# pierluigiferrari/fcn8s_tensorflow

Hardware: AMD Instinct MI355X
Metric: training images/sec at 1024x512 bs16 (higher is better)
Workload: dtype f32; 1 GPU; FCN-8s (VGG-16, fc6 7x7, 20 classes) train step, 1024x512, 16 images/GPU, SGD+momentum, keep_prob 0.5; global_batch=16, parallelism=dp1

## Files before the change

fcn8s_tensorflow_amd/csrc/conv_route.h:

```cpp
#pragma once
#include <algorithm>

namespace fcn8s {

struct RouteOpts {
    int wino_min_cin = 64;
    int wino_tile = 6;
    int wino_tile_hires = 0, wino_hires_pixels = 0;
    int wino_force_tile = 0;
    int wino_fc6 = 1;
    int plan_N = 0;
    bool scratch = false;
};
struct ConvShape { int N, H, W, Cin, Cout, K; };
inline ConvShape transposed(ConvShape s) { std::swap(s.Cin, s.Cout); return s; }

inline int wino_tile_for(const RouteOpts& o, int H, int W, int K = 3)
{
    if (H % 2 || W % 2) return 0;
    if (o.wino_force_tile && K == 3) return (o.wino_force_tile == 6 || (H % o.wino_force_tile == 0 && W % o.wino_force_tile == 0)) ? o.wino_force_tile : 0;
    int tmax = o.wino_tile;
    if (K == 3 && o.wino_tile_hires && o.wino_hires_pixels > 0 && (long long)H * W >= o.wino_hires_pixels && o.wino_tile_hires < tmax) tmax = o.wino_tile_hires;
    const bool t4 = tmax >= 4 && H % 4 == 0 && W % 4 == 0;
    if (K == 7) return (o.wino_tile >= 4 && H % 4 == 0 && W % 4 == 0) ? 4 : 0;
// ... 29 lines not shown
inline RbWriter relu_record_writer(const RouteOpts& o, const ConvShape& l, const ConvShape& next, bool l_is_conv1_1)
{
    if (l_is_conv1_1 && l.Cout % 64 == 0 && keeps_v(o, next)) return RbWriter::consumer;
    return keeps_v(o, l) ? RbWriter::self : RbWriter::none;
}
inline bool out_in_fused(const RouteOpts& o, const ConvShape& l, const ConvShape& next) { return l.K == 3 && next.K == 3 && fwd_tile(o, l) == 6 && fwd_tile(o, next) == 6; }
inline bool conv1_in_next_transform(const RouteOpts& o, const ConvShape& conv1_1, const ConvShape& next) { return conv1_1.Cout == 64 && fwd_tile(o, next) == 6; }
inline bool dm_from_next(const RouteOpts& o, const ConvShape& l)
{
    return o.scratch && keeps_v(o, l) && wino_tile_for(o, l.H, l.W, 3) == 6 && l.Cin % 64 == 0 && l.Cout % 64 == 0;
}
inline bool pool_in_transform(const RouteOpts& o, const ConvShape& last, bool has_prev)
{
    return o.wino_min_cin > 0 && last.Cout >= o.wino_min_cin && o.scratch && wino_tile_for(o, last.H, last.W, 3) >= 4 && last.Cout % 64 == 0 && has_prev && keeps_v(o, last);
}

struct Bf16Opts {
    bool acts = true;
    bool fuse_pool = true;
    bool conv1_tiled = true;
    bool copies = true;
};
inline bool bf16_kernels_take(const ConvShape& s) { return s.Cin % 64 == 0 && s.Cout % 64 == 0 && s.K % 2 == 1; }
inline bool pool_feeds_skip(int block) { return block == 3 || block == 4; }
inline bool bf16_plane_fits(long long plane_elems) { return (double)plane_elems * 2.0 + 65536.0 < 4294967296.0; }

inline bool conv1_writes_bf16_only(const Bf16Opts& o, const ConvShape& conv1_1, const ConvShape& next)
{
    return o.copies && o.acts && o.conv1_tiled && conv1_1.H % 8 == 0 && conv1_1.W % 16 == 0 && conv1_1.Cout % 64 == 0 && bf16_kernels_take(next);
}
// ... 26 lines not shown
```

fcn8s_tensorflow_amd/csrc/fcn8s_internal.h:

```cpp
#pragma once
#include <hip/hip_runtime.h>
#include <stdint.h>
#include <cmath>
#include "../../include/fcn8s_hip.h"

#if defined(__HIP_DEVICE_COMPILE__) && !defined(__gfx950__)
#error "libfcn8s_hip is written for gfx950 (MI355X) only: build with --offload-arch=gfx950"
#endif
#define FCN8S_LDS_BYTES_NEEDED (160u * 1024u)

#include <string>
namespace fcn8s {

extern thread_local const char* g_last_kernel;
void defer_error(int code, const char* fmt, ...) __attribute__((format(printf, 2, 3)));
int take_deferred_error(std::string* text);

struct IgemmArgs {
    const float* x; const float* w; const float* bias; const float* addend; const float* mask;
    float* y;
    int N, Ma, Mb; long long M;
    int Hi, Wi, Cin, ldx;
    int KW, in_scale, tap_step, tap_off, Ktot;
    int Ho, Wo, Cout, ldy;
// ... 187 lines not shown
inline float tf_adam_lr_t(float lr, float b1, float b2, long long t)
{
    return lr * (float)std::sqrt(1.0 - std::pow((double)b2, (double)t)) / (float)(1.0 - std::pow((double)b1, (double)t));
}
void launch_ema_update(float* sh, const float* theta, long long n, float w, const int* ok_dev, hipStream_t s);
void launch_swap(float* a, float* b, long long n, hipStream_t s);
void launch_flip_transpose(const float* w, float* wt, int taps, int Cin, int Cout, hipStream_t s);
void launch_pad_cin(const float* w, float* w4, int taps, int Cin, int Cinp, int Cout, hipStream_t s);
void launch_tconv_phase_pack(const float* w, float* wp, int K, int S, int C, hipStream_t s);
void launch_dropout_mask(float* mask, long long n, float keep_prob, unsigned long long seed,
                         unsigned int stream_id, hipStream_t s);
int wino_r(int KS);
int wino_nsub(int KS);
int wino_alpha(int tile, int KS);
long long wino_slab(long long T, int C);
void launch_wino_filter(int tile, const float* w, float* u, int Cin, int Cout, int KS, hipStream_t s, int transpose_out = 0);
void launch_wino_input(int tile, const float* x, float* v, int N, int H, int W, int C, int KS, hipStream_t s, unsigned* rbits_out = nullptr);
void launch_wino_input_conv1(const float* x0, const float* w4, const float* bias, float* v, int N, int H, int W, hipStream_t s, unsigned* rbits_out = nullptr);
void launch_wino_input_xb(const float* x, float* v, unsigned short* xb, int N, int H, int W, int C, hipStream_t s, unsigned* rbits_out = nullptr);
bool launch_wino_input_dout(int tile, const float* dy, float* v, float* dm, int N, int H, int W, int C, hipStream_t s, const unsigned char* pidx = nullptr);
void launch_wino_output(int tile, const float* m, const float* bias, const float* addend, const float* mask, float mask_scale,
                        int relu, float* y, int N, int H, int W, int C, int dropout, float keep, unsigned long long seed,
                        unsigned int stream_id, hipStream_t s, float* pool = nullptr, unsigned char* pidx = nullptr, int KS = 3,
                        unsigned* rbits_out = nullptr, const unsigned* rbits_in = nullptr);
size_t wino_rbits_words(int tile, int N, int H, int W, int C);
void launch_wino_dout(int tile, const float* dy, float* dm, int N, int H, int W, int C, hipStream_t s, int KS = 3, const unsigned char* pidx = nullptr);
void launch_wino_dgrad_output_dout(const float* dv, const unsigned* rbits_in, float* dm, int N, int H, int W, int C, hipStream_t s);
void launch_wino_dgrad_output_sub44(const float* dv, float* dx, int N, int H, int W, int C, hipStream_t s);
void launch_wino_dgrad_output(const float* dv, const float* addend, const float* mask, float mask_scale, const unsigned* rbits_in, float* y,
                              int N, int H, int W, int C, hipStream_t s);
bool launch_wino_out_in(const float* m, const float* bias, float* v, unsigned* rbits_out, int N, int H, int W, int C, hipStream_t s, bool always = false);
// ... 81 lines not shown
```

fcn8s_tensorflow_amd/csrc/model.hip:

```cpp
#include "../../include/fcn8s_hip.h"
#include "fcn8s_internal.h"
#include "device_buffer.h"
#include "pass_state.h"
#include "conv_route.h"
#include <cstdarg>
#include <functional>

#include <dlfcn.h>
#include <atomic>
#include <chrono>
#include <thread>
#include <cmath>
#include <cstdio>
#include <cstring>
#include <cstdlib>
#include <algorithm>
#include <mutex>
#include <map>
#include <set>
#include <string>
#include <vector>

using namespace fcn8s;

// ... 31 lines not shown
struct Act { float* p = nullptr; size_t n = 0; int H = 0, W = 0, C = 0; };

const int kConvsPerBlock[5] = {2, 2, 3, 3, 3};

struct Layer {
    char name[8], pool_name[8], pool_in[12];
    int block, pos, nconv;
    int h, w, cin, cout, K, real_cin;
    int prev, next;
    size_t w_off, b_off;
    int i_y, i_rb, i_wv, i_pool, i_pidx;
    float *y, *wv, *pool; unsigned* rb; unsigned char* pidx;
    int tile;
    RbWriter rb_writer;
    bool out_in_next, conv1_in_next;
    bool dm_from_next, pool_in_transform;
    ConvShape shape(int N) const { return ConvShape{N, h, w, cin, cout, K}; }
    bool first() const { return real_cin != 0; }
    bool last_of_block() const { return pos == nconv; }
};

}

namespace fcn8s {
void defer_error(int code, const char* fmt, ...)
{
    if (t_deferred_code) return;
    char buf[1024];
    va_list ap; va_start(ap, fmt); vsnprintf(buf, sizeof buf, fmt, ap); va_end(ap);
    t_deferred_code = code; t_deferred_text = buf;
}
// ... 40 lines not shown
    int wino_tile_hires = 0, wino_hires_pixels = 0;
    int wino_force_tile = 0;
    int precision = FCN8S_PREC_F32;
    bool frozen = false;
    unsigned long long frozen_fp = 0; DeviceBuf<unsigned long long> d_fp;
    PinnedBuf<unsigned long long> h_fp; hipEvent_t fp_event = nullptr;
    std::map<std::string, DeviceBuf<float>> u_cache;
    std::map<std::string, DeviceBuf<float>> u_train;
    bool fwd_train = false;
    PassState pass;
    int deterministic = 0;
    int fuse_dgrad_dout = 1;
    int fuse_out_in = 1;
    int conv1_tiled = 1, conv1_wgrad_mfma = 1;
    int conv1_in_transform = 1;
    DeviceBuf<unsigned short> d_wbf16;
    std::map<std::string, DeviceBuf<unsigned short>> wbf16_cache;
    std::set<std::string> bank_stale; bool banks_stale = false;
    int bf16_gemm256 = 1;
    DeviceBuf<unsigned short> d_abf16;
    std::map<std::string, DeviceBuf<unsigned short>> xbf16;
    using G16Map = std::map<std::string, DeviceBuf<unsigned short>>;
    G16Map xg16, dyg16;
    std::set<std::string> g16_stale;
    int bf16_fuse_pool = 1;
    int bf16_infer_copies = 1;
    int bf16_rows_bn = 0;
    int bf16_acts = 1;
    bool fp8_calibrated = false; float fp8_amax[FCN8S_FP8_LAYERS] = {}; DeviceBuf<unsigned> d_fp8_amax;
    std::map<std::string, Q8Buf> q8;
// ... 182 lines not shown

static void prof_derived(fcn8s_model* m, const char* what)
{
    if (m && m->profile && m->profile_detail) m->groups[group_id(m, (std::string("derived:") + what).c_str())].launches += 1;
}

struct ConvEpi { float alpha = 1.f; };
struct FwdEpi : ConvEpi {
    const float* bias = nullptr; int relu = 0;
    int dropout = 0; float keep = 1.f; uint32_t stream_id = 0;
    float* pool_out = nullptr; unsigned char* pool_idx = nullptr;
    int skip_y = 0;
    unsigned* relu_bits_out = nullptr;
    unsigned* in_relu_bits_out = nullptr; const char* in_layer = nullptr;
    float* next_v = nullptr; const char* next_layer = nullptr;
};
struct DgradEpi : ConvEpi {
    const float* addend = nullptr;
    const float* mask = nullptr; float mask_scale = 1.f;
    const unsigned* relu_bits_in = nullptr;
    const float* w_fwd = nullptr;
    int lazy_wt = 0;
    float* dm_out = nullptr; const char* dm_out_layer = nullptr;
    const char* yb_layer = nullptr; int yb_K = 3;
    bool yb_only = false;
};

thread_local int t_op_split = 0;
thread_local int t_op_rows_bn = 0;
thread_local int t_op_planes = 1;
// ... 22 lines not shown
    o.wino_min_cin = m->wino_min_cin; o.wino_tile = m->wino_tile; o.wino_tile_hires = m->wino_tile_hires; o.wino_hires_pixels = m->wino_hires_pixels;
    o.wino_force_tile = m->wino_force_tile; o.wino_fc6 = m->wino_fc6; o.plan_N = m->plan_N; o.scratch = m->d_wino_v != nullptr;
    return o;
}
int wino_tile_for(const fcn8s_model* m, int H, int W, int K = 3) { return m ? wino_tile_for(route_opts(m), H, W, K) : 0; }
Bf16Opts bf16_opts(const fcn8s_model* m, bool train)
{
    Bf16Opts o; o.acts = m->bf16_acts != 0; o.fuse_pool = m->bf16_fuse_pool != 0; o.conv1_tiled = m->conv1_tiled != 0; o.copies = train || m->bf16_infer_copies != 0;
    return o;
}
long long wino_tiles(int tile, int N, int H, int W) { return (long long)N * ((H + tile - 1) / tile) * ((W + tile - 1) / tile); }
struct WinoEpi { const float* bias = nullptr; const float* addend = nullptr; const float* mask = nullptr; float mask_scale = 1.f;
                 int relu = 0; int dropout = 0; float keep = 1.f; unsigned long long seed = 0; unsigned int stream_id = 0; float* pool = nullptr; unsigned char* pidx = nullptr;
                 unsigned* rbits_out = nullptr; const unsigned* rbits_in = nullptr; int skip_y = 0;
                 unsigned* in_rbits_out = nullptr;
                 float* next_v = nullptr; bool* fused_out = nullptr; };
static bool fft6_cheaper(const fcn8s_model* m, int H, int W)
{
    const long long fft = 292LL * ((H + 7) / 8) * ((W + 7) / 8);
    const long long other = wino_tile_for(m, H, W, 7) == 4 ? 196LL * (H / 4) * (W / 4) : 49LL * H * W;
    return fft < other;
}
static bool fft6_shape_ok(const fcn8s_model* m, int ci, int co) { return m->wino_fc6 && m->fc6_fft && m->fc6k == 7 && ci % 16 == 0 && co % 128 == 0; }
static bool fft6_on(const fcn8s_model* m, int N, int H, int W, int ci, int co)
{
    if (!m || !fft6_shape_ok(m, ci, co) || !fft6_cheaper(m, H, W) || m->precision != FCN8S_PREC_F32 || m->frozen || !m->d_wino_v || !m->d_wino_m) return false;
    const long long T = fft_fc6_tiles(N, H, W);
    auto v = m->acts.find("wino_v"), mm = m->acts.find("wino_m");
    return v != m->acts.end() && mm != m->acts.end() && v->second.n >= (size_t)fft_fc6_planes() * (size_t)wino_slab(T, ci) &&
           mm->second.n >= std::max((size_t)fft_fc6_planes() * (size_t)wino_slab(T, co), (size_t)T * 196 * ci);
}
// ... 96 lines not shown
    a.fixed_tile = 1; a.bt = 1; a.ldw = Cdy;
    { ProfScope ps(m, "fc6_fft_gemm_dgrad", 2.0 * P * T * Cdy * Cdx, 4.0 * P * (T * (double)(Cdy + Cdx) + (double)Cdy * Cdx), layer); launch_igemm(a, P, s); }
    { ProfScope ps(m, "fc6_fft_transform", 0, 4.0 * ((double)P * T * Cdx + 2.0 * 196.0 * T * Cdx + (double)N * H * W * Cdx));
      launch_fft_fc6_din(m->d_wino_v, m->d_wino_m, dx, N, H, W, Cdx, s); }
}

void conv_winograd(fcn8s_model* m, int tile, int KS, bool fwd, const float* x, const float* wk, float* y, float* u, float* v, float* mm,
                   int N, int H, int W, int Cin, int Cout, const WinoEpi& e, hipStream_t s, const char* layer, bool v_ready = false)
{
    const int P = wino_alpha(tile, KS) * wino_alpha(tile, KS), nsub2 = wino_nsub(KS) * wino_nsub(KS);
    const long long T = wino_tiles(tile, N, H, W);
    const int Kg = nsub2 * Cin;
    IgemmArgs a = position_gemm(v, u, mm, T, Kg, Cout); a.split = split_of(m);
    const double tb = 4.0 * ((double)N * H * W * Cin * nsub2 + (double)P * T * Kg), ob = 4.0 * ((double)N * H * W * Cout * ((e.pool ? (e.skip_y ? 0.25 : 1.25) : 1.0) + (e.rbits_in ? 1.0 / 32 : (e.mask ? 1.0 : 0.0)) + (e.addend ? 1.0 : 0.0) + (e.rbits_out ? 1.0 / 32 : 0.0)) + (double)P * T * Cout);
    bool u_cached = false;
    const char* tag = KS == 7 ? (fwd ? "wino_gemm_fc6_fwd" : "wino_gemm_fc6_dgrad") : (fwd ? "wino_gemm_fwd" : "wino_gemm_dgrad");
    if (m && m->frozen && layer && fwd) {
        DeviceBuf<float>& cu = m->u_cache[std::string(layer) + "#" + std::to_string(tile)];
        const std::string key = "u:" + std::string(layer) + "#" + std::to_string(tile);
        if (cu && !m->bank_stale.count(key)) { u = cu; u_cached = true; }
        else if (cu) { u = cu; m->bank_stale.erase(key); }
        else if (cu.grow((size_t)P * Kg * Cout * sizeof(float), s, &m->ws_allocs)) u = cu;
        a.w = u;
    }
    if (m && !u_cached && m->fwd_train && layer && fwd && ((KS == 3 && tile == 6) || (KS == 7 && tile == 4))) {
        DeviceBuf<float>& tu = m->u_train[std::string(layer) + "#" + std::to_string(tile)];
        if (tu.grow((size_t)P * Kg * Cout * sizeof(float), s)) { u = tu; a.w = u; }
    }
    auto pre = [&]() { if (!u_cached) { prof_derived(m, "wino_filter_kernel"); launch_wino_filter(tile, wk, u, Cin, Cout, KS, s); } if (!v_ready) launch_wino_input(tile, x, v, N, H, W, Cin, KS, s, e.in_rbits_out); };
    auto post = [&]() {
        if (e.next_v && tile == 6 && KS == 3 && e.relu && e.bias && !e.addend && !e.mask && !e.dropout && !e.pool && !e.rbits_in &&
            launch_wino_out_in(mm, e.bias, e.next_v, e.rbits_out, N, H, W, Cout, s, m && m->fuse_out_in >= 2)) { if (e.fused_out) *e.fused_out = true; return; }
        launch_wino_output(tile, mm, e.bias, e.addend, e.mask, e.mask_scale, e.relu, (e.skip_y && e.pool) ? nullptr : y, N, H, W, Cout, e.dropout, e.keep, e.seed, e.stream_id, s, e.pool, e.pidx, KS, e.rbits_out, e.rbits_in); };
    const double ob_fused = 4.0 * (2.0 * P * T * Cout + (e.rbits_out ? (double)N * H * W * Cout / 32 : 0.0));
    { ProfScope ps(m, "wino_transform", 0, (v_ready ? 0.0 : tb) + (u_cached ? 0.0 : (double)(KS * KS + P * nsub2) * 4 * Cin * Cout)); pre(); }
    { ProfScope ps(m, tag, 2.0 * P * T * Kg * Cout, 4.0 * P * (T * (double)(Kg + Cout) + (double)Kg * Cout), layer); launch_igemm(a, P, s); }
    { ProfScope ps(m, "wino_transform", 0, ob); post(); if (e.fused_out && *e.fused_out && m && m->profile && !m->groups.empty()) { const int g = group_id(m, "wino_transform"); m->groups[g].bytes += ob_fused - ob; } }
}

static void conv_direct(fcn8s_model* m, const char* group, IgemmArgs a, const float* x, const float* w, float* y,
                        int N, int H, int W, int Cin, int Cout, int K, hipStream_t s, int real_cin, const char* layer)
{
    a.split = split_of(m);
    a.x = x; a.w = w; a.y = y;
    a.N = N; a.Ma = H; a.Mb = W; a.M = (long long)N * H * W;
    a.Hi = H; a.Wi = W; a.Cin = Cin; a.ldx = Cin;
    a.KW = K; a.in_scale = 1; a.tap_step = 1; a.tap_off = -(K - 1) / 2; a.Ktot = K * K * Cin;
    a.Ho = H; a.Wo = W; a.Cout = Cout; a.ldy = Cout;
    a.out_scale = 1; a.out_offy = 0; a.out_offx = 0; a.phases_x = 1; a.w_phase_stride = 0;
    a.seed = m ? m->seed : 0;
// ... 18 lines not shown
        conv_fft6_fwd(m, layer, x, w, y, N, H, W, Cin, Cout, e.bias, e.relu, e.dropout, e.keep, e.stream_id, s)) return false;
    if (m) m->pass.drop_backward_handoffs();
    const int tile = fwd_tile(route_opts(m), ConvShape{N, H, W, Cin, Cout, K});
    if (tile && !(K == 3 && e.dropout) && e.alpha == 1.f && !real_cin) {
        const bool v_ready = m->pass.fwd_v.take(layer);
        m->pass.fwd_v.drop();
        float* vbuf = m->d_wino_v;
        if (layer) { auto it = m->acts.find(std::string("wv:") + layer); if (it != m->acts.end()) vbuf = it->second.p; }
        WinoEpi we; we.bias = e.bias; we.relu = e.relu;
        we.dropout = e.dropout; we.keep = e.keep; we.seed = m->seed; we.stream_id = e.stream_id; we.pool = e.pool_out; we.pidx = e.pool_idx;
        we.rbits_out = e.relu_bits_out; we.skip_y = e.skip_y && e.pool_out;
        if (e.relu_bits_out && layer) m->pass.rbits_ok.insert(layer);
        if (e.in_relu_bits_out && e.in_layer && K == 3) { we.in_rbits_out = e.in_relu_bits_out; m->pass.rbits_ok.insert(e.in_layer); }
        bool fused_out = false;
        if (e.next_v && e.next_layer) { we.next_v = e.next_v; we.fused_out = &fused_out; }
        conv_winograd(m, tile, K, true, x, w, y, m->d_wino_u, vbuf, m->d_wino_m, N, H, W, Cin, Cout, we, s, layer, v_ready);
        if (fused_out) { m->pass.fwd_v.give(e.next_layer); if (layer) m->pass.y_unwritten.insert(layer); }
        return e.pool_out != nullptr;
    }
    IgemmArgs a{}; a.bias = e.bias; a.alpha = e.alpha; a.relu = e.relu; a.mask_scale = 1.f; a.dropout = e.dropout; a.keep_prob = e.keep; a.stream_id = e.stream_id;
    conv_direct(m, group, a, x, w, y, N, H, W, Cin, Cout, K, s, real_cin, layer);
    return false;
}

struct BwdCall {
    fcn8s_model* m;
    hipStream_t s;
    const char* layer;
    const char* group;
    ConvShape fwd;
// ... 372 lines not shown
    fill_layer_table(m, H, W, pl.layers);
    size_t vmax = 0, gmax = 0;
    std::vector<size_t> n_rb(pl.layers.size(), 0), n_wv(pl.layers.size(), 0);
    for (size_t k = 0; k < pl.layers.size(); ++k) {
        Layer& L = pl.layers[k];
        gmax = std::max(gmax, (size_t)N * L.h * L.w * L.cout);
        if (L.block > 5) continue;
        const ConvShape sh = L.shape(N);
        const Layer* nx = in_block_next(pl.layers, L);
        L.tile = wino_tile_for(ro, L.h, L.w, 3);
        L.rb_writer = nx ? relu_record_writer(ro, sh, nx->shape(N), L.first()) : RbWriter::none;
        L.out_in_next = nx && out_in_fused(ro, sh, nx->shape(N));
        L.conv1_in_next = L.first() && nx && nx->last_of_block() && conv1_in_next_transform(ro, sh, nx->shape(N));
        L.dm_from_next = nx && dm_from_next(ro, sh);
        L.pool_in_transform = L.last_of_block() && pool_in_transform(ro, sh, in_block_prev(pl.layers, L) != nullptr);
        if (L.rb_writer != RbWriter::none) n_rb[k] = wino_rbits_words(L.tile, N, L.h, L.w, L.cout);
        if (keeps_v(ro, sh)) n_wv[k] = slab_floats(L.h, L.w, L.cin, 3);
        if (const int c = scratch_channels(ro, sh)) vmax = std::max(vmax, slab_floats(L.h, L.w, c, 3));
    }
    add("x0", H, W, 4);
    for (Layer& L : pl.layers) {
        if (L.block > 5) break;
        L.i_y = add(L.name, L.h, L.w, L.cout);
        if (L.last_of_block()) { const int ip = add(L.pool_name, L.h / 2, L.w / 2, L.cout); for (int k = 0; k < L.nconv; ++k) (&L - k)->i_pool = ip; }
    }
    const int h5 = H / 32, w5 = W / 32, h4 = H / 16, w4 = W / 16, h3 = H / 8, w3 = W / 8;
    for (size_t k = 0; k < pl.layers.size(); ++k) if (n_rb[k]) pl.layers[k].i_rb = add_raw(std::string("rb:") + pl.layers[k].name, n_rb[k]);
    for (Layer& L : pl.layers)
        if (L.block <= 5 && L.last_of_block()) {
            const int ip = add_raw("pidx" + std::to_string(L.block), ((size_t)N * (L.h / 2) * (L.w / 2) * (size_t)L.cout + 3) / 4);
// ... 523 lines not shown
    return FwdStep{};
}

static FwdStep fwd_conv(fcn8s_model* m, Layer& L, const float* x, bool train)
{
    const Layer* nx = in_block_next(m->layers, L);
    FwdEpi e; e.bias = m->d_params + L.b_off; e.relu = 1;
    if (train && L.rb_writer == RbWriter::self) e.relu_bits_out = L.rb;
    if (train && L.pos == 2 && m->layers[L.prev].rb_writer == RbWriter::consumer) {
        e.in_relu_bits_out = m->layers[L.prev].rb; e.in_layer = m->layers[L.prev].name;
    }
    if (L.last_of_block()) {
        e.pool_out = L.pool;
        if (train) e.pool_idx = L.pidx;
        e.skip_y = !train || L.pool_in_transform;
    }
    if (L.out_in_next && m->fuse_out_in && !(bf16_fwd_mode(m) && L.block >= 3) && !bf16_train_mode(m) && !fp8_mode(m) && (!train || e.relu_bits_out)) {
        e.next_v = nx->wv ? nx->wv : m->d_wino_v; e.next_layer = nx->name;
    }
    FwdStep st;
    const float* wt = L.first() ? m->d_w1pad : m->d_params + L.w_off;
    st.pooled = conv_fwd(m, L.first() ? "conv1_1_fwd" : "conv3x3_fwd", x, wt, L.y, m->N, L.h, L.w, L.cin, L.cout, 3, e, m->stream, L.real_cin, L.name);
    return st;
}

static FwdStep fwd_pool(fcn8s_model* m, const Layer& L, const Layer& cons, const float* x, bool train, bool fp8, bool pooled, const Bf16Opts& bo)
{
    hipStream_t s = m->stream; const int N = m->N, b = L.block - 1, h = L.h, w = L.w, cin = L.cout; const char* pn = L.pool_name;
    if (fp8) {
        m->pass.pool_fused[b] = false; m->pass.pool_routed[b] = false;
// ... 710 lines not shown
    if (key == "winograd_min_cin") return &m->wino_min_cin;
    if (key == "winograd_tile") return &m->wino_tile;
    if (key == "winograd_fc6") return &m->wino_fc6;
    if (key == "fc6_fft") return &m->fc6_fft;
    if (key == "fc6_fft_wgrad") return &m->fc6_fft_wgrad;
    if (key == "tconv_gemm") return &m->tconv_gemm;
    if (key == "fuse_dgrad_dout") return &m->fuse_dgrad_dout;
    if (key == "fuse_out_in") return &m->fuse_out_in;
    if (key == "bf16_gemm256") return &m->bf16_gemm256;
    if (key == "winograd_tile_hires") return &m->wino_tile_hires;
    if (key == "winograd_hires_pixels") return &m->wino_hires_pixels;
    if (key == "conv1_tiled") return &m->conv1_tiled;
    if (key == "conv1_wgrad_mfma") return &m->conv1_wgrad_mfma;
    if (key == "bf16_copy_by_transform") return &m->bf16_copy_by_transform;
    if (key == "conv1_in_transform") return &m->conv1_in_transform;
    if (key == "deterministic") return &m->deterministic;
    if (key == "bf16_acts") return &m->bf16_acts;
    if (key == "bf16_rows_bn") return &m->bf16_rows_bn;
    if (key == "keep_output_gradients") return &m->keep_dy;
    if (key == "bf16_infer_copies") return &m->bf16_infer_copies;
    if (key == "bf16_fuse_pool") return &m->bf16_fuse_pool;
    return nullptr;
}
int fcn8s_set_option(fcn8s_model* m, const char* key, int64_t value)
{
    if (!key) return fail(m, FCN8S_ERR_BAD_ARG, "fcn8s_set_option: null key");
    const std::string k = key;
    if (k == "device_bytes_live" || k == "scratch_bytes_live") return fail(m, FCN8S_ERR_BAD_ARG, "fcn8s_set_option: '" + k + "' is read-only");
    if (!m) {
        if (k == "op_f32x3") { t_op_split = value ? 3 : 0; return FCN8S_OK; }
// ... 2051 lines not shown
```

fcn8s_tensorflow_amd/csrc/winograd.hip:

```cpp
#include "fcn8s_internal.h"
#include <cstdlib>

namespace fcn8s {

static inline int wcap(long long work)
{
    long long b = (work + 255) / 256;
    return (int)(b > 4096 ? 4096 : (b < 1 ? 1 : b));
}

template <int M, int R = 3> struct WinoMat;
template <> struct WinoMat<2, 3> {
    static constexpr int A = 4;
    static __device__ __forceinline__ float bt(int i, int j) { constexpr float m[4][4] = {{1, 0, -1, 0}, {0, 1, 1, 0}, {0, -1, 1, 0}, {0, 1, 0, -1}}; return m[i][j]; }
    static __device__ __forceinline__ float g(int i, int j) { constexpr float m[4][3] = {{1, 0, 0}, {.5f, .5f, .5f}, {.5f, -.5f, .5f}, {0, 0, 1}}; return m[i][j]; }
    static __device__ __forceinline__ float at(int i, int j) { constexpr float m[2][4] = {{1, 1, 1, 0}, {0, 1, -1, -1}}; return m[i][j]; }
};
template <> struct WinoMat<4, 3> {
    static constexpr int A = 6;
    static __device__ __forceinline__ float bt(int i, int j)
    {
        constexpr float m[6][6] = {{4, 0, -5, 0, 1, 0}, {0, -4, -4, 1, 1, 0}, {0, 4, -4, -1, 1, 0},
                                   {0, -2, -1, 2, 1, 0}, {0, 2, -1, -2, 1, 0}, {0, 4, 0, -5, 0, 1}};
        return m[i][j];
// ... 88 lines not shown
    const bool odd = threadIdx.x & 1;
    const VecF<2> send = odd ? s0 : s1;
    VecF<2> got; got.d[0] = __shfl_xor(send.d[0], 1); got.d[1] = __shfl_xor(send.d[1], 1);
    VecF<4> o;
    if (!odd) { o.d[0] = s0.d[0]; o.d[1] = s0.d[1]; o.d[2] = got.d[0]; o.d[3] = got.d[1]; }
    else { o.d[0] = got.d[0]; o.d[1] = got.d[1]; o.d[2] = s1.d[0]; o.d[3] = s1.d[1]; }
    VecF<4>* dst = reinterpret_cast<VecF<4>*>(odd ? p - 1 + slab : p);
    if constexpr (NT) vstore_nt<4>(dst, o); else *dst = o;
    __builtin_amdgcn_sched_barrier(0);
}
#define f4fma vfma<VEC>
#define f4zero vzero<VEC>
#define VF VecF<VEC>

template <int M, int R>
__global__ void wino_filter_kernel(const float* w, float* u, int Cin, int Cout, int KS, int nsub, int transpose_out)
{
    constexpr int A = WinoMat<M, R>::A;
    const long long cc = (long long)Cin * Cout, total = cc * nsub * nsub, ucc = cc * nsub * nsub;
    for (long long i0 = blockIdx.x * (long long)blockDim.x + threadIdx.x; i0 < total; i0 += (long long)gridDim.x * blockDim.x) {
        const long long i = transpose_out ? (i0 % Cin) * Cout + i0 / Cin : i0;
        const int sub = (int)(i / cc); const long long e = i - sub * cc;
        const int sa = sub / nsub, sb = sub - sa * nsub;
        float g[R][R], t[A][R];
#pragma unroll
        for (int a = 0; a < R; ++a)
#pragma unroll
            for (int b = 0; b < R; ++b) {
                const int ky = R * sa + a, kx = R * sb + b;
                g[a][b] = (ky < KS && kx < KS) ? w[(long long)(ky * KS + kx) * cc + e] : 0.f;
            }
// ... 2 lines not shown
#pragma unroll
            for (int b = 0; b < R; ++b) {
                float s = 0.f;
#pragma unroll
                for (int k = 0; k < R; ++k) s = fmaf(WinoMat<M, R>::g(a, k), g[k][b], s);
                t[a][b] = s;
            }
#pragma unroll
        for (int a = 0; a < A; ++a)
#pragma unroll
            for (int b = 0; b < A; ++b) {
                float s = 0.f;
#pragma unroll
                for (int k = 0; k < R; ++k) s = fmaf(t[a][k], WinoMat<M, R>::g(b, k), s);
                u[(long long)(a * A + b) * ucc + (transpose_out ? i0 : i)] = s;
            }
    }
}

struct TileIdx { int n, ty, tx, c; long long t; bool ok; };
static __device__ __forceinline__ TileIdx tile_index(int th, int tw, int C4, int N)
{
    TileIdx r;
    const unsigned bx = blockIdx.x, by = blockIdx.y;
    const int idx = bx * 256 + threadIdx.x;
    r.tx = idx / C4; r.c = idx - r.tx * C4;
    r.n = by / th; r.ty = by - r.n * th;
    r.ok = r.tx < tw && r.n < N;
    r.t = ((long long)r.n * th + r.ty) * tw + r.tx;
    return r;
// ... 895 lines not shown
#undef VF

int wino_r(int KS) { return KS == 3 ? 3 : 4; }
int wino_nsub(int KS) { const int r = wino_r(KS); return (KS + r - 1) / r; }
size_t wino_rbits_words(int tile, int N, int H, int W, int C)
{
    const int vec = tile == 2 ? 4 : 2;
    const size_t T = (size_t)N * ((H + tile - 1) / tile) * ((W + tile - 1) / tile);
    return T * (size_t)(C / vec) * (size_t)((tile * tile * vec + 31) / 32);
}
int wino_alpha(int tile, int KS) { return tile + (tile == 6 ? 3 : wino_r(KS)) - 1; }
long long wino_slab(long long T, int C)
{
    return T * C + 1088;
}
void launch_wino_filter(int tile, const float* w, float* u, int Cin, int Cout, int KS, hipStream_t s, int transpose_out)
{
    const int nsub = wino_nsub(KS);
    const int g = wcap((long long)Cin * Cout * nsub * nsub);
    if (nsub != 1) transpose_out = 0;
    if (tile == 6)                    hipLaunchKernelGGL((wino_filter_kernel<6, 3>), dim3(g), dim3(256), 0, s, w, u, Cin, Cout, KS, nsub, transpose_out);
    else if (tile == 4 && wino_r(KS) == 4) hipLaunchKernelGGL((wino_filter_kernel<4, 4>), dim3(g), dim3(256), 0, s, w, u, Cin, Cout, KS, nsub, transpose_out);
    else if (tile == 4)               hipLaunchKernelGGL((wino_filter_kernel<4, 3>), dim3(g), dim3(256), 0, s, w, u, Cin, Cout, KS, nsub, transpose_out);
    else                              hipLaunchKernelGGL((wino_filter_kernel<2, 3>), dim3(g), dim3(256), 0, s, w, u, Cin, Cout, KS, nsub, transpose_out);
}
void launch_wino_dgrad_output(const float* dv, const float* addend, const float* mask, float mask_scale, const unsigned* rbits_in, float* y,
                              int N, int H, int W, int C, hipStream_t s)
{
    constexpr int M_ = 6;
    const long long T = (long long)N * ((H + M_ - 1) / M_) * ((W + M_ - 1) / M_);
    hipLaunchKernelGGL((wino_dgrad_output_kernel<2>), tile_grid(N, (H + M_ - 1) / M_, (W + M_ - 1) / M_, C / 2), dim3(256), 0, s,
                       (const VecF<2>*)dv, (const VecF<2>*)addend, (const VecF<2>*)mask, mask_scale, rbits_in, (VecF<2>*)y, N, H, W, C / 2, wino_slab(T, C) / 2);
}
void launch_wino_dgrad_output_dout(const float* dv, const unsigned* rbits_in, float* dm, int N, int H, int W, int C, hipStream_t s)
{
    constexpr int M_ = 6;
    const long long T = (long long)N * ((H + M_ - 1) / M_) * ((W + M_ - 1) / M_);
    g_last_kernel = "wino_dgrad_output_dout_kernel<2>";
    hipLaunchKernelGGL((wino_dgrad_output_dout_kernel<2>), tile_grid(N, (H + M_ - 1) / M_, (W + M_ - 1) / M_, C / 2), dim3(256), 0, s,
// ... 113 lines not shown
```

Before: 298.5 images/sec.

## Fuse Winograd GEMM, output transform, bias, ReLU and maxpool for conv1_2

Adds a dedicated MFMA kernel for the 64->64 F(6,3) Winograd conv1_2 forward pass. It does the batched GEMM in registers, stages results through LDS, and applies the inverse transform, bias, ReLU and 2x2 max-pool with argmax in the same kernel. This removes the round trip of the large transformed-output tensor M through global memory and the separate output-transform launch at the highest-resolution layer. The filter transform also writes a second copy of U pre-swizzled for the MFMA layout. The cost is a 512-thread, one-block-per-CU kernel using large LDS, which limits occupancy.

```diff
diff --git a/fcn8s_tensorflow_amd/csrc/conv_route.h b/fcn8s_tensorflow_amd/csrc/conv_route.h
--- a/fcn8s_tensorflow_amd/csrc/conv_route.h
+++ b/fcn8s_tensorflow_amd/csrc/conv_route.h
@@ -67,6 +67,10 @@
 {
     return o.wino_min_cin > 0 && last.Cout >= o.wino_min_cin && o.scratch && wino_tile_for(o, last.H, last.W, 3) >= 4 && last.Cout % 64 == 0 && has_prev && keeps_v(o, last);
 }
+inline bool gemm_out_fused64(const RouteOpts& o, const ConvShape& last, bool has_prev, bool last_is_conv1_2)
+{
+    return last_is_conv1_2 && last.K == 3 && last.Cin == 64 && last.Cout == 64 && fwd_tile(o, last) == 6 && pool_in_transform(o, last, has_prev);
+}
 
 struct Bf16Opts {
     bool acts = true;
diff --git a/fcn8s_tensorflow_amd/csrc/fcn8s_internal.h b/fcn8s_tensorflow_amd/csrc/fcn8s_internal.h
--- a/fcn8s_tensorflow_amd/csrc/fcn8s_internal.h
+++ b/fcn8s_tensorflow_amd/csrc/fcn8s_internal.h
@@ -225,7 +225,9 @@
 int wino_nsub(int KS);
 int wino_alpha(int tile, int KS);
 long long wino_slab(long long T, int C);
-void launch_wino_filter(int tile, const float* w, float* u, int Cin, int Cout, int KS, hipStream_t s, int transpose_out = 0);
+void launch_wino_filter(int tile, const float* w, float* u, int Cin, int Cout, int KS, hipStream_t s, int transpose_out = 0, float* u_mfma64 = nullptr);
+bool launch_wino_gemm_out64(const float* v, const float* u_mfma64, const float* bias, float* pool, unsigned char* pidx, int N, int H, int W, hipStream_t s);
+size_t wino_gemm_out64_bank_floats();
 void launch_wino_input(int tile, const float* x, float* v, int N, int H, int W, int C, int KS, hipStream_t s, unsigned* rbits_out = nullptr);
 void launch_wino_input_conv1(const float* x0, const float* w4, const float* bias, float* v, int N, int H, int W, hipStream_t s, unsigned* rbits_out = nullptr);
 void launch_wino_input_xb(const float* x, float* v, unsigned short* xb, int N, int H, int W, int C, hipStream_t s, unsigned* rbits_out = nullptr);
diff --git a/fcn8s_tensorflow_amd/csrc/model.hip b/fcn8s_tensorflow_amd/csrc/model.hip
--- a/fcn8s_tensorflow_amd/csrc/model.hip
+++ b/fcn8s_tensorflow_amd/csrc/model.hip
@@ -69,7 +69,7 @@
     int tile;
     RbWriter rb_writer;
     bool out_in_next, conv1_in_next;
-    bool dm_from_next, pool_in_transform;
+    bool dm_from_next, pool_in_transform, gemm_out_fused64;
     ConvShape shape(int N) const { return ConvShape{N, h, w, cin, cout, K}; }
     bool first() const { return real_cin != 0; }
     bool last_of_block() const { return pos == nconv; }
@@ -140,6 +140,7 @@
     int fuse_out_in = 1;
     int conv1_tiled = 1, conv1_wgrad_mfma = 1;
     int conv1_in_transform = 1;
+    int gemm_out_fused64 = 1;
     DeviceBuf<unsigned short> d_wbf16;
     std::map<std::string, DeviceBuf<unsigned short>> wbf16_cache;
     std::set<std::string> bank_stale; bool banks_stale = false;
@@ -352,6 +353,7 @@
     unsigned* relu_bits_out = nullptr;
     unsigned* in_relu_bits_out = nullptr; const char* in_layer = nullptr;
     float* next_v = nullptr; const char* next_layer = nullptr;
+    bool gemm_out_fused64 = false;
 };
 struct DgradEpi : ConvEpi {
     const float* addend = nullptr;
@@ -404,7 +406,8 @@
                  int relu = 0; int dropout = 0; float keep = 1.f; unsigned long long seed = 0; unsigned int stream_id = 0; float* pool = nullptr; unsigned char* pidx = nullptr;
                  unsigned* rbits_out = nullptr; const unsigned* rbits_in = nullptr; int skip_y = 0;
                  unsigned* in_rbits_out = nullptr;
-                 float* next_v = nullptr; bool* fused_out = nullptr; };
+                 float* next_v = nullptr; bool* fused_out = nullptr;
+                 bool gemm_out_fused64 = false; };
 static bool fft6_cheaper(const fcn8s_model* m, int H, int W)
 {
     const long long fft = 292LL * ((H + 7) / 8) * ((W + 7) / 8);
@@ -531,26 +534,37 @@
     IgemmArgs a = position_gemm(v, u, mm, T, Kg, Cout); a.split = split_of(m);
     const double tb = 4.0 * ((double)N * H * W * Cin * nsub2 + (double)P * T * Kg), ob = 4.0 * ((double)N * H * W * Cout * ((e.pool ? (e.skip_y ? 0.25 : 1.25) : 1.0) + (e.rbits_in ? 1.0 / 32 : (e.mask ? 1.0 : 0.0)) + (e.addend ? 1.0 : 0.0) + (e.rbits_out ? 1.0 / 32 : 0.0)) + (double)P * T * Cout);
     bool u_cached = false;
+    const size_t bank = (size_t)P * Kg * Cout;
+    const bool bank2 = m && layer && fwd && e.gemm_out_fused64 && tile == 6 && KS == 3 && Cin == 64 && Cout == 64;
+    const size_t bank_bytes = (bank + (bank2 ? wino_gemm_out64_bank_floats() : 0)) * sizeof(float);
+    size_t u_floats = m && u == m->d_wino_u ? m->ufl : bank;
     const char* tag = KS == 7 ? (fwd ? "wino_gemm_fc6_fwd" : "wino_gemm_fc6_dgrad") : (fwd ? "wino_gemm_fwd" : "wino_gemm_dgrad");
     if (m && m->frozen && layer && fwd) {
         DeviceBuf<float>& cu = m->u_cache[std::string(layer) + "#" + std::to_string(tile)];
         const std::string key = "u:" + std::string(layer) + "#" + std::to_string(tile);
-        if (cu && !m->bank_stale.count(key)) { u = cu; u_cached = true; }
-        else if (cu) { u = cu; m->bank_stale.erase(key); }
-        else if (cu.grow((size_t)P * Kg * Cout * sizeof(float), s, &m->ws_allocs)) u = cu;
+        if (cu && !m->bank_stale.count(key)) { u = cu; u_cached = true; u_floats = cu.elems(); }
+        else if (cu) { u = cu; u_floats = cu.elems(); m->bank_stale.erase(key); }
+        else if (cu.grow(bank_bytes, s, &m->ws_allocs)) { u = cu; u_floats = cu.elems(); }
         a.w = u;
     }
     if (m && !u_cached && m->fwd_train && layer && fwd && ((KS == 3 && tile == 6) || (KS == 7 && tile == 4))) {
         DeviceBuf<float>& tu = m->u_train[std::string(layer) + "#" + std::to_string(tile)];
-        if (tu.grow((size_t)P * Kg * Cout * sizeof(float), s)) { u = tu; a.w = u; }
-    }
-    auto pre = [&]() { if (!u_cached) { prof_derived(m, "wino_filter_kernel"); launch_wino_filter(tile, wk, u, Cin, Cout, KS, s); } if (!v_ready) launch_wino_input(tile, x, v, N, H, W, Cin, KS, s, e.in_rbits_out); };
+        if (tu.grow(bank_bytes, s)) { u = tu; a.w = u; u_floats = tu.elems(); }
+    }
+    float* const u64 = bank2 && u_floats >= bank + wino_gemm_out64_bank_floats() ? u + bank : nullptr;
+    const bool gemm_out64 = u64 && m->precision == FCN8S_PREC_F32 && split_of(m) == 0 && e.pool && e.skip_y && e.bias && e.relu && !e.addend && !e.mask && !e.dropout && !e.rbits_in && !e.rbits_out && !e.next_v;
+    auto pre = [&]() { if (!u_cached) { prof_derived(m, "wino_filter_kernel"); launch_wino_filter(tile, wk, u, Cin, Cout, KS, s, 0, u64); } if (!v_ready) launch_wino_input(tile, x, v, N, H, W, Cin, KS, s, e.in_rbits_out); };
     auto post = [&]() {
         if (e.next_v && tile == 6 && KS == 3 && e.relu && e.bias && !e.addend && !e.mask && !e.dropout && !e.pool && !e.rbits_in &&
             launch_wino_out_in(mm, e.bias, e.next_v, e.rbits_out, N, H, W, Cout, s, m && m->fuse_out_in >= 2)) { if (e.fused_out) *e.fused_out = true; return; }
         launch_wino_output(tile, mm, e.bias, e.addend, e.mask, e.mask_scale, e.relu, (e.skip_y && e.pool) ? nullptr : y, N, H, W, Cout, e.dropout, e.keep, e.seed, e.stream_id, s, e.pool, e.pidx, KS, e.rbits_out, e.rbits_in); };
     const double ob_fused = 4.0 * (2.0 * P * T * Cout + (e.rbits_out ? (double)N * H * W * Cout / 32 : 0.0));
-    { ProfScope ps(m, "wino_transform", 0, (v_ready ? 0.0 : tb) + (u_cached ? 0.0 : (double)(KS * KS + P * nsub2) * 4 * Cin * Cout)); pre(); }
+    { ProfScope ps(m, "wino_transform", 0, (v_ready ? 0.0 : tb) + (u_cached ? 0.0 : (double)(KS * KS + P * nsub2 + (u64 ? P : 0)) * 4 * Cin * Cout)); pre(); }
+    if (gemm_out64) {
+        ProfScope ps(m, tag, 2.0 * P * T * Kg * Cout, 4.0 * P * (T * (double)Kg + (double)Kg * Cout) + (double)N * H * W * Cout * (1.0 + (e.pidx ? 0.25 : 0.0)), layer);
+        if (!launch_wino_gemm_out64(v, u64, e.bias, e.pool, e.pidx, N, H, W, s)) defer_error(FCN8S_ERR_HIP, "wino_gemm_out64_kernel could not be launched for %s (%d x %d x %d)", layer, N, H, W);
+        return;
+    }
     { ProfScope ps(m, tag, 2.0 * P * T * Kg * Cout, 4.0 * P * (T * (double)(Kg + Cout) + (double)Kg * Cout), layer); launch_igemm(a, P, s); }
     { ProfScope ps(m, "wino_transform", 0, ob); post(); if (e.fused_out && *e.fused_out && m && m->profile && !m->groups.empty()) { const int g = group_id(m, "wino_transform"); m->groups[g].bytes += ob_fused - ob; } }
 }
@@ -599,6 +613,7 @@
         if (e.in_relu_bits_out && e.in_layer && K == 3) { we.in_rbits_out = e.in_relu_bits_out; m->pass.rbits_ok.insert(e.in_layer); }
         bool fused_out = false;
         if (e.next_v && e.next_layer) { we.next_v = e.next_v; we.fused_out = &fused_out; }
+        we.gemm_out_fused64 = e.gemm_out_fused64;
         conv_winograd(m, tile, K, true, x, w, y, m->d_wino_u, vbuf, m->d_wino_m, N, H, W, Cin, Cout, we, s, layer, v_ready);
         if (fused_out) { m->pass.fwd_v.give(e.next_layer); if (layer) m->pass.y_unwritten.insert(layer); }
         return e.pool_out != nullptr;
@@ -1001,6 +1016,7 @@
         L.conv1_in_next = L.first() && nx && nx->last_of_block() && conv1_in_next_transform(ro, sh, nx->shape(N));
         L.dm_from_next = nx && dm_from_next(ro, sh);
         L.pool_in_transform = L.last_of_block() && pool_in_transform(ro, sh, in_block_prev(pl.layers, L) != nullptr);
+        L.gemm_out_fused64 = L.last_of_block() && gemm_out_fused64(ro, sh, in_block_prev(pl.layers, L) != nullptr, L.block == 1);
         if (L.rb_writer != RbWriter::none) n_rb[k] = wino_rbits_words(L.tile, N, L.h, L.w, L.cout);
         if (keeps_v(ro, sh)) n_wv[k] = slab_floats(L.h, L.w, L.cin, 3);
         if (const int c = scratch_channels(ro, sh)) vmax = std::max(vmax, slab_floats(L.h, L.w, c, 3));
@@ -1554,6 +1570,7 @@
         e.pool_out = L.pool;
         if (train) e.pool_idx = L.pidx;
         e.skip_y = !train || L.pool_in_transform;
+        e.gemm_out_fused64 = L.gemm_out_fused64 && m->gemm_out_fused64;
     }
     if (L.out_in_next && m->fuse_out_in && !(bf16_fwd_mode(m) && L.block >= 3) && !bf16_train_mode(m) && !fp8_mode(m) && (!train || e.relu_bits_out)) {
         e.next_v = nx->wv ? nx->wv : m->d_wino_v; e.next_layer = nx->name;
@@ -2294,6 +2311,7 @@
     if (key == "conv1_wgrad_mfma") return &m->conv1_wgrad_mfma;
     if (key == "bf16_copy_by_transform") return &m->bf16_copy_by_transform;
     if (key == "conv1_in_transform") return &m->conv1_in_transform;
+    if (key == "gemm_out_fused64") return &m->gemm_out_fused64;
     if (key == "deterministic") return &m->deterministic;
     if (key == "bf16_acts") return &m->bf16_acts;
     if (key == "bf16_rows_bn") return &m->bf16_rows_bn;
diff --git a/fcn8s_tensorflow_amd/csrc/wino_fused64.hip b/fcn8s_tensorflow_amd/csrc/wino_fused64.hip
--- /dev/null
+++ b/fcn8s_tensorflow_amd/csrc/wino_fused64.hip
@@ -0,0 +1,137 @@
+#include "fcn8s_internal.h"
+
+namespace fcn8s {
+
+typedef float f32x4 __attribute__((ext_vector_type(4)));
+
+static __device__ __forceinline__ float at63(int i, int j)
+{
+    constexpr float m[6][8] = {{1, 1, 1, 1, 1, 1, 1, 0}, {0, 1, -1, 2, -2, 1.f / 2, -1.f / 2, 0}, {0, 1, 1, 4, 4, 1.f / 4, 1.f / 4, 0},
+                               {0, 1, -1, 8, -8, 1.f / 8, -1.f / 8, 0}, {0, 1, 1, 16, 16, 1.f / 16, 1.f / 16, 0}, {0, 1, -1, 32, -32, 1.f / 32, -1.f / 32, 1}};
+    return m[i][j];
+}
+
+constexpr int kF64Tiles = 16;
+constexpr int kF64Lt = 33;
+constexpr int kF64Dist = 2;
+constexpr size_t kF64LdsBytes = (size_t)64 * kF64Tiles * kF64Lt * sizeof(float);
+
+template <bool NT>
+__global__ __launch_bounds__(512, 1) void wino_gemm_out64_kernel(const float* __restrict__ v, const float* __restrict__ up, const float* __restrict__ bias,
+                                                                 float* __restrict__ pool, unsigned char* __restrict__ pidx,
+                                                                 int N, int H, int W, long long T, long long slab)
+{
+    extern __shared__ float lds[];
+    constexpr int D = kF64Dist, LT = kF64Lt;
+    const int tid = threadIdx.x, lane = tid & 63, wave = __builtin_amdgcn_readfirstlane(tid >> 6);
+    const long long t0 = (long long)blockIdx.x * kF64Tiles;
+    const int ti = lane & 15, q = lane >> 4;
+    f32x4 acc[8][4];
+#pragma unroll
+    for (int i = 0; i < 8; ++i)
+#pragma unroll
+        for (int j = 0; j < 4; ++j) acc[i][j] = (f32x4){0.f, 0.f, 0.f, 0.f};
+    const long long trow = t0 + ti < T ? t0 + ti : T - 1;
+    const float* vbase = v + (long long)(8 * wave) * slab + trow * 64 + q * 4;
+    const float* ubase = up + (long long)(8 * wave) * 4096 + lane * 4;
+    f32x4 ra[D + 1], rb[D + 1][4];
+    auto issue = [&](int g) {
+        const int npi = g >> 2, nkc = g & 3, sl = g % (D + 1);
+        ra[sl] = *reinterpret_cast<const f32x4*>(vbase + npi * slab + nkc * 16);
+#pragma unroll
+        for (int nb = 0; nb < 4; ++nb) rb[sl][nb] = *reinterpret_cast<const f32x4*>(ubase + ((npi * 4 + nkc) * 4 + nb) * 256);
+    };
+#pragma unroll
+    for (int g = 0; g < D; ++g) issue(g);
+#pragma unroll
+    for (int g = 0; g < 32; ++g) {
+        if (g + D < 32) issue(g + D);
+        __builtin_amdgcn_sched_barrier(0);
+        const int pi = g >> 2, sl = g % (D + 1);
+#pragma unroll
+        for (int s = 0; s < 4; ++s)
+#pragma unroll
+            for (int nb = 0; nb < 4; ++nb) acc[pi][nb] = __builtin_amdgcn_mfma_f32_16x16x4f32(ra[sl][s], rb[sl][nb][s], acc[pi][nb], 0, 0, 0);
+        __builtin_amdgcn_sched_barrier(0);
+    }
+    const int tl = tid >> 5, c = tid & 31;
+    const int th = (H + 5) / 6, tw = (W + 5) / 6, Hp = H / 2, Wp = W / 2;
+    const long long t = t0 + tl;
+    const bool ok = t < T;
+    const long long tc = ok ? t : T - 1;
+    const int n = (int)(tc / ((long long)th * tw)), rem = (int)(tc - (long long)n * th * tw), ty = rem / tw, tx = rem - ty * tw;
+#pragma unroll
+    for (int half = 0; half < 2; ++half) {
+        if (half) __syncthreads();
+#pragma unroll
+        for (int pi = 0; pi < 8; ++pi)
+#pragma unroll
+            for (int nb2 = 0; nb2 < 2; ++nb2)
+#pragma unroll
+                for (int r = 0; r < 4; ++r) lds[((8 * wave + pi) * kF64Tiles + 4 * q + r) * LT + 16 * nb2 + ti] = acc[pi][2 * half + nb2][r];
+        __syncthreads();
+        const int ch = 32 * half + c;
+        const float* mp = lds + tl * LT + c;
+        float qv[6][8];
+#pragma unroll
+        for (int b = 0; b < 8; ++b) {
+            float col[8];
+#pragma unroll
+            for (int a = 0; a < 8; ++a) col[a] = mp[(a * 8 + b) * kF64Tiles * LT];
+#pragma unroll
+            for (int o = 0; o < 6; ++o) {
+                float s = 0.f;
+#pragma unroll
+                for (int k = 0; k < 8; ++k) if (at63(o, k) != 0.f) s = fmaf(at63(o, k), col[k], s);
+                qv[o][b] = s;
+            }
+        }
+        const float bv = bias[ch];
+        float pmax[3][3]; unsigned char parg[3][3];
+#pragma unroll
+        for (int oy = 0; oy < 6; ++oy)
+#pragma unroll
+            for (int ox = 0; ox < 6; ++ox) {
+                float y = bv;
+#pragma unroll
+                for (int k = 0; k < 8; ++k) if (at63(ox, k) != 0.f) y = fmaf(at63(ox, k), qv[oy][k], y);
+                const int py = oy / 2, px = ox / 2;
+                const bool inside = 6 * ty + oy < H && 6 * tx + ox < W;
+                if (!inside) { if ((oy & 1) == 0 && (ox & 1) == 0) { pmax[py][px] = y; parg[py][px] = 0; } continue; }
+                y = fmaxf(y, 0.f);
+                if ((oy & 1) == 0 && (ox & 1) == 0) { pmax[py][px] = y; parg[py][px] = 0; }
+                else if (y > pmax[py][px]) { pmax[py][px] = y; parg[py][px] = (unsigned char)((oy & 1) * 2 + (ox & 1)); }
+            }
+        if (ok) {
+#pragma unroll
+            for (int py = 0; py < 3; ++py)
+#pragma unroll
+                for (int px = 0; px < 3; ++px)
+                    if (3 * ty + py < Hp && 3 * tx + px < Wp) {
+                        const long long po = (((long long)n * Hp + 3 * ty + py) * Wp + 3 * tx + px) * 64 + ch;
+                        if constexpr (NT) __builtin_nontemporal_store(pmax[py][px], pool + po); else pool[po] = pmax[py][px];
+                        if (pidx) pidx[po] = pmax[py][px] > 0.f ? parg[py][px] : (unsigned char)4;
+                    }
+        }
+    }
+}
+
+size_t wino_gemm_out64_bank_floats() { return (size_t)64 * 64 * 64; }
+
+bool launch_wino_gemm_out64(const float* v, const float* up, const float* bias, float* pool, unsigned char* pidx, int N, int H, int W, hipStream_t s)
+{
+    if (!v || !up || !bias || !pool || N <= 0 || H <= 0 || W <= 0 || H % 2 || W % 2) return false;
+    const long long T = (long long)N * ((H + 5) / 6) * ((W + 5) / 6);
+    const long long blocks = (T + kF64Tiles - 1) / kF64Tiles;
+    if (blocks > 0x7fffffffLL) return false;
+    const bool big = (double)N * H * W * 64 >= 64e6;
+    const hipError_t e = hipFuncSetAttribute(big ? reinterpret_cast<const void*>(&wino_gemm_out64_kernel<true>) : reinterpret_cast<const void*>(&wino_gemm_out64_kernel<false>),
+                                             hipFuncAttributeMaxDynamicSharedMemorySize, (int)kF64LdsBytes);
+    if (e != hipSuccess) { defer_error(FCN8S_ERR_HIP, "wino_gemm_out64: %zu bytes of LDS refused (%s)", kF64LdsBytes, hipGetErrorString(e)); return false; }
+    g_last_kernel = "wino_gemm_out64_kernel";
+    if (big) hipLaunchKernelGGL(wino_gemm_out64_kernel<true>, dim3((unsigned)blocks), dim3(512), kF64LdsBytes, s, v, up, bias, pool, pidx, N, H, W, T, wino_slab(T, 64));
+    else     hipLaunchKernelGGL(wino_gemm_out64_kernel<false>, dim3((unsigned)blocks), dim3(512), kF64LdsBytes, s, v, up, bias, pool, pidx, N, H, W, T, wino_slab(T, 64));
+    return true;
+}
+
+}
diff --git a/fcn8s_tensorflow_amd/csrc/winograd.hip b/fcn8s_tensorflow_amd/csrc/winograd.hip
--- a/fcn8s_tensorflow_amd/csrc/winograd.hip
+++ b/fcn8s_tensorflow_amd/csrc/winograd.hip
@@ -126,7 +126,7 @@
 #define VF VecF<VEC>
 
 template <int M, int R>
-__global__ void wino_filter_kernel(const float* w, float* u, int Cin, int Cout, int KS, int nsub, int transpose_out)
+__global__ void wino_filter_kernel(const float* w, float* u, int Cin, int Cout, int KS, int nsub, int transpose_out, float* u_mfma64)
 {
     constexpr int A = WinoMat<M, R>::A;
     const long long cc = (long long)Cin * Cout, total = cc * nsub * nsub, ucc = cc * nsub * nsub;
@@ -159,6 +159,8 @@
 #pragma unroll
                 for (int k = 0; k < R; ++k) s = fmaf(t[a][k], WinoMat<M, R>::g(b, k), s);
                 u[(long long)(a * A + b) * ucc + (transpose_out ? i0 : i)] = s;
+                if (u_mfma64) { const int ci = (int)(e / Cout), co = (int)(e - (long long)ci * Cout);
+                                u_mfma64[(a * A + b) * 4096 + ((((ci >> 4) * 4 + (co >> 4)) * 64 + ((ci >> 2) & 3) * 16 + (co & 15)) << 2) + (ci & 3)] = s; }
             }
     }
 }
@@ -1084,15 +1086,17 @@
 {
     return T * C + 1088;
 }
-void launch_wino_filter(int tile, const float* w, float* u, int Cin, int Cout, int KS, hipStream_t s, int transpose_out)
+void launch_wino_filter(int tile, const float* w, float* u, int Cin, int Cout, int KS, hipStream_t s, int transpose_out, float* u_mfma64)
 {
     const int nsub = wino_nsub(KS);
     const int g = wcap((long long)Cin * Cout * nsub * nsub);
     if (nsub != 1) transpose_out = 0;
-    if (tile == 6)                    hipLaunchKernelGGL((wino_filter_kernel<6, 3>), dim3(g), dim3(256), 0, s, w, u, Cin, Cout, KS, nsub, transpose_out);
-    else if (tile == 4 && wino_r(KS) == 4) hipLaunchKernelGGL((wino_filter_kernel<4, 4>), dim3(g), dim3(256), 0, s, w, u, Cin, Cout, KS, nsub, transpose_out);
-    else if (tile == 4)               hipLaunchKernelGGL((wino_filter_kernel<4, 3>), dim3(g), dim3(256), 0, s, w, u, Cin, Cout, KS, nsub, transpose_out);
-    else                              hipLaunchKernelGGL((wino_filter_kernel<2, 3>), dim3(g), dim3(256), 0, s, w, u, Cin, Cout, KS, nsub, transpose_out);
+    if (tile != 6 || KS != 3 || Cin != 64 || Cout != 64 || transpose_out) u_mfma64 = nullptr;
+    float* const no64 = nullptr;
+    if (tile == 6)                    hipLaunchKernelGGL((wino_filter_kernel<6, 3>), dim3(g), dim3(256), 0, s, w, u, Cin, Cout, KS, nsub, transpose_out, u_mfma64);
+    else if (tile == 4 && wino_r(KS) == 4) hipLaunchKernelGGL((wino_filter_kernel<4, 4>), dim3(g), dim3(256), 0, s, w, u, Cin, Cout, KS, nsub, transpose_out, no64);
+    else if (tile == 4)               hipLaunchKernelGGL((wino_filter_kernel<4, 3>), dim3(g), dim3(256), 0, s, w, u, Cin, Cout, KS, nsub, transpose_out, no64);
+    else                              hipLaunchKernelGGL((wino_filter_kernel<2, 3>), dim3(g), dim3(256), 0, s, w, u, Cin, Cout, KS, nsub, transpose_out, no64);
 }
 void launch_wino_dgrad_output(const float* dv, const float* addend, const float* mask, float mask_scale, const unsigned* rbits_in, float* y,
                               int N, int H, int W, int C, hipStream_t s)
```

Result: faster. 301.8 images/sec, median of 6 (+1.1%).
